# xavi-pinsach/kzg-grandsums-study

Hardware: AMD Instinct MI355X
Metric: grand-sum proofs/sec + MSM G1-adds/sec at n=2^20, 1/2/4/8 MI355X (higher is better)
Workload: dtype u32 limbs (BN254 Fr/Fq Montgomery: 8 x 32-bit; MSM buckets 9 x 29-bit), int VALU; 1 GPU; grandsum prover, n=2^20, k=1, no selectors, inputs resident in HBM; nbits=20, npols=1, selectors=False, parallelism=replicas x1, inflight_per_gpu=4, srs_power=20, srs_points_resident=2097151

## Files before the change

include/kgs.h:

```cpp
#ifndef KGS_H
#define KGS_H
#include <stddef.h>
#include <stdint.h>

#ifdef __cplusplus
extern "C" {
#endif

#define KGS_OK 0
#define KGS_E_ARG (-1)
#define KGS_E_HIP (-2)
#define KGS_E_NOT_WELL_CALC (-3)
#define KGS_E_NOT_DIVISIBLE (-4)
#define KGS_E_DOES_NOT_DIVIDE (-5)
#define KGS_E_IO (-6)
#define KGS_E_SRS (-7)
#define KGS_E_COMM (-8)
#define KGS_E_RANGE (-9)
#define KGS_E_NOT_IN_TABLE (-10)

#define KGS_GRANDSUM 0
#define KGS_GRANDPRODUCT 1
#define KGS_LOOKUP 2

// ... 3 lines not shown
const char* kgs_version(void);

int kgs_device_count(int* count);
int kgs_ctx_create(int device, kgs_ctx_t** out);
void kgs_ctx_destroy(kgs_ctx_t* ctx);

typedef int (*kgs_allgather_fn)(void* user, const uint8_t* send, uint8_t* recv, uint64_t bytes);
int kgs_ctx_set_shard(kgs_ctx_t* ctx, int rank, int world, kgs_allgather_fn fn, void* user);
int kgs_shard_range(uint64_t n, int rank, int world, uint64_t* lo, uint64_t* hi);
int kgs_msm_combine(const uint8_t* T_all, int nparts, int c, uint8_t out_lem[64]);

typedef struct kgs_group kgs_group_t;
int kgs_group_create_local(int world, kgs_group_t** out);
int kgs_group_create_host(int world, kgs_allgather_fn fn, void* user, kgs_group_t** out);
typedef int (*kgs_alltoall_fn)(void* user, const uint8_t* send, uint8_t* recv, uint64_t chunk);
int kgs_group_create_host_a2a(int world, kgs_allgather_fn fn, kgs_alltoall_fn a2a, void* user, kgs_group_t** out);
int kgs_group_rccl_unique_id(uint8_t id[128]);
int kgs_group_create_rccl(int rank, int world, const uint8_t id[128], int device, kgs_group_t** out);
void kgs_group_destroy(kgs_group_t* g);
int kgs_group_world(kgs_group_t* g, int* world);
int kgs_ctx_set_group(kgs_ctx_t* ctx, kgs_group_t* g, int rank);
int kgs_last_exchange(kgs_ctx_t* ctx, double* out, int max);

int kgs_ctx_set_msm_lanes(kgs_ctx_t* ctx, int lanes);

int kgs_ctx_set_reference_quirks(kgs_ctx_t* ctx, int on);

int kgs_srs_load_ptau(kgs_ctx_t* ctx, const char* path, int nbits_max);
int kgs_srs_load_ptau_slice(kgs_ctx_t* ctx, const char* path, int nbits_max, int rank, int world);
int kgs_srs_slice_info(kgs_ctx_t* ctx, int* rank, int* world, uint64_t* table_bytes);
int kgs_ptau_power(const char* path, int* power);
int kgs_srs_load_points(kgs_ctx_t* ctx, const uint8_t* g1_lem, uint64_t npts, int power, int nbits_max);
int kgs_srs_info(kgs_ctx_t* ctx, int* power, uint64_t* npts, int* window_c);
int kgs_ptau_read_tau_g2(const char* path, uint8_t out128[128]);

int kgs_ptau_write_synthetic(kgs_ctx_t* ctx, const char* path, int power, const uint8_t tau_std[32]);

int kgs_prove(kgs_ctx_t* ctx, int kind, int nbits, int npols, const uint8_t* const* evals_f,
              const uint8_t* const* evals_t, const uint8_t* sel_f, const uint8_t* sel_t, uint8_t* const* mont_f,
              uint8_t* const* mont_t, uint8_t* commitments_out, uint8_t* evaluations_out);
int kgs_host_register(void* ptr, uint64_t bytes);
int kgs_host_unregister(void* ptr);
int kgs_ctx_idle(kgs_ctx_t* ctx);
int kgs_prove_device(kgs_ctx_t* ctx, int kind, int nbits, int npols, const void* const* d_evals_f,
                     const void* const* d_evals_t, const void* d_sel_f, const void* d_sel_t, uint8_t* commitments_out,
                     uint8_t* evaluations_out);
int kgs_proof_shape(int kind, int npols, int selected, int* n_commitments, int* n_evaluations);

int kgs_verify(int kind, int nbits, int npols, int selected, const uint8_t* commitments, const uint8_t* evaluations,
               const uint8_t tau_g2[128]);
int kgs_verify_ptau(int kind, const char* ptau_path, int nbits, int npols, int selected, const uint8_t* commitments,
                    const uint8_t* evaluations);
int kgs_pairing_eq(int npairs, const uint8_t* g1_lem, const uint8_t* g2_lem);

typedef struct {
  int kind, nbits, npols, selected;
  const uint8_t* commitments;
  const uint8_t* evaluations;
} kgs_proof_ref_t;
typedef struct {
  uint8_t* weights_out;
  uint8_t* folded_out;
  uint32_t pairing_checks;
  uint32_t terms;
  int on_gpu;
  double fold_ms, pairing_ms;
// ... 85 lines not shown
```

kzg-grandsums-study_amd/csrc/field29.hpp:

```cpp
#pragma once
#include "field.hpp"

#ifndef KGS_M32_ROWS
#define KGS_M32_ROWS 8
#endif
#ifndef KGS_M32_ROWS_MUL2
#define KGS_M32_ROWS_MUL2 8
#endif
static_assert(KGS_M32_ROWS <= 8 && KGS_M32_ROWS_MUL2 <= 8, "column bounds of fq29::reduce_row32");

namespace kgs {
namespace f29 {

constexpr uint32_t MASK = 0x1fffffffu;
constexpr uint32_t INV = 0x04866389u;
constexpr uint32_t INV32 = 0x24866389u;
struct L9 {
  uint32_t v[9];
};
constexpr L9 Q = {{0x187cfd47u, 0x010460b6u, 0x1c72a34fu, 0x02d522d0u, 0x1585d978u, 0x02db40c0u, 0x00a6e141u,
                   0x0e5c2634u, 0x0030644eu}};
constexpr L9 ONE = {{0x157ccc21u, 0x141c2758u, 0x185230d3u, 0x014c0419u, 0x0aa36fb9u, 0x1d4240ceu, 0x11d54c07u,
                     0x052ac7a8u, 0x000dc836u}};
constexpr L9 C256 = {{0x058f0d9du, 0x1aea1c6eu, 0x11c2cf74u, 0x11d651ebu, 0x1462c0a7u, 0x11b7bc3cu, 0x1cbd99bau,
// ... 185 lines not shown
      const int64_t s = (int64_t)(Kc.v[j] - b.l[j]) + (int64_t)x.t[j] + c;
      r.l[j] = j < 8 ? ((uint32_t)s & f29::MASK) : (uint32_t)s;
      c = s >> 29;
    }
    return r;
  }

  __device__ __forceinline__ static fq29 mul(const fq29& a, const fq29& b) { return carry(mul_cols(a, b)); }
  __device__ __forceinline__ static fq29 sqr(const fq29& a) { return carry(sqr_cols(a)); }
  __device__ __forceinline__ static fq29 mul2(const fq29& a, const fq29& b, const fq29& c2, const fq29& d2) {
    return carry(mul2_cols(a, b, c2, d2));
  }

  __device__ __forceinline__ bool maybe_zero8() const {
    return ((l[0] * (0u - f29::INV)) & f29::MASK) < 8u;
  }
  __device__ __forceinline__ fq to_fq() const {
    fq29 m = mul(*this, from(f29::C256));
    fq r;
    m.pack(r.v);
    return fq::reduce_once(r);
  }
  __device__ __forceinline__ static fq29 from_fq(const fq& a) { return mul(unpack(a.v), from(f29::C266)); }
};

constexpr int RAW29_WORDS = 40;

struct g1_acc29 {
  fq29 X, Y, ZZ, ZZZ;
  bool inf;

  __device__ __forceinline__ void set_inf() { inf = true; }

  __device__ __forceinline__ void add_aff(const uint32_t* xw, const uint32_t* yw, bool negy) {
    uint32_t z = 0;
#pragma unroll
    for (int i = 0; i < 8; i++) z |= xw[i] | yw[i];
    if (z == 0) return;
    const fq29 x2 = fq29::unpack(xw), y2 = fq29::unpack(yw);
    if (inf) {
      X = x2;
      const fq29 yn = fq29::neg<2, 1>(y2).norm();
#pragma unroll
      for (int j = 0; j < 9; j++) Y.l[j] = negy ? yn.l[j] : y2.l[j];
      ZZ = fq29::from(f29::ONE);
      ZZZ = ZZ;
      inf = false;
      return;
    }
    const fq29 P = fq29::carry_sub<30, 1>(fq29::mul_cols(x2, ZZ), X);
    const fq29 S2 = fq29::mul(y2, ZZZ);
    fq29 R = fq29::neg<32, 2>(Y);
#pragma unroll
    for (int j = 0; j < 9; j++) R.l[j] = negy ? R.l[j] - S2.l[j] : R.l[j] + S2.l[j];
    R = R.norm();
    const fq29 PP = fq29::sqr(P);
    if (PP.maybe_zero8()) {
      if (P.to_fq().is_zero()) {
        if (R.to_fq().is_zero()) {
          g1_aff a;
          a.x = x2.to_fq();
          a.y = y2.to_fq();
          if (negy) a.y = a.y.neg();
          const g1_xyzz d = g1_xyzz::dbl_aff(a);
          X = fq29::from_fq(d.X);
          Y = fq29::from_fq(d.Y);
          ZZ = fq29::from_fq(d.ZZ);
          ZZZ = fq29::from_fq(d.ZZZ);
        } else {
          inf = true;
        }
// ... 100 lines not shown
```

kzg-grandsums-study_amd/csrc/kernels.hpp:

```cpp
#pragma once

#ifndef KGS_NO_PRIO_AUX
#define KGS_AUX_PRIO() __builtin_amdgcn_s_setprio(3)
#else
#define KGS_AUX_PRIO() ((void)0)
#endif

#include <hip/hip_runtime.h>
#include <stdint.h>
#include "field.hpp"

namespace kgs {

constexpr int LC_MAX = 32;
constexpr int LC_W29 = 10;
struct LinComb {
  int nterms;
  const uint32_t* src[LC_MAX];
  uint64_t len[LC_MAX];
  uint32_t coef[LC_MAX][8];
  uint32_t coef29[LC_MAX][LC_W29];
  uint32_t c0[8];
};

constexpr int EB_MAX = 32;
struct EvalBatch {
  int npolys;
  const uint32_t* src[EB_MAX];
  uint64_t len[EB_MAX];
};

struct MsmTables {
  uint32_t* table = nullptr;
  uint64_t npts = 0;
  int c = 0, W = 0;
};

constexpr int MSM_SL_G_MAX = 128;
constexpr int MSM_NH_MAX = 2048;
inline int msm_lob(int c) {
  int lob = c - 1 < 7 ? c - 1 : 7;
  if (c - 9 > lob) lob = c - 9 > 8 ? 8 : c - 9;
  return lob;
}
inline int msm_nh(int c) { return (1 << (c - 1)) >> msm_lob(c); }
struct MsmWork {
  int32_t* digit = nullptr;
  uint8_t* lo = nullptr;
  uint32_t* blockhist = nullptr;
  uint32_t *counts = nullptr, *offsets = nullptr, *cursor = nullptr, *sorted = nullptr;
  uint32_t* part = nullptr;
  uint32_t* segowner = nullptr;
  uint32_t* locnt = nullptr;
  uint32_t* chunklist = nullptr;
  uint32_t* chunkcnt = nullptr;
  uint32_t* raw29 = nullptr;
};

bool ntt_set_coresident(bool on);
constexpr int TW29_WORDS = 10;
void ntt_register_tw29(const uint32_t* base, uint64_t count, const uint32_t* twin);
void ntt_unregister_tw29(const uint32_t* base);
void launch_tw29(hipStream_t st, uint32_t* out, const uint32_t* in, uint64_t count);
void ntt_dif(hipStream_t st, uint32_t* out, const uint32_t* in, uint64_t in_len, int logm, const uint32_t* pre,
             const uint32_t* tw, int logM);
void ntt_dit(hipStream_t st, uint32_t* out, const uint32_t* in, int in_bitrev, int logm, const uint32_t* tw, int logM,
             const uint32_t* post, const uint32_t* post_s);
void launch_powers(hipStream_t st, uint32_t* out, uint64_t count, const uint32_t* w_dev, const uint32_t* scale_dev);
// ... 40 lines not shown
                           uint64_t N, uint64_t rot);
void launch_ref_divzh(hipStream_t st, uint32_t* c, uint64_t n, uint32_t ext, uint32_t* flag);

void launch_gather_e(hipStream_t st, uint32_t* out, const uint32_t* in, uint64_t N, int W, int r, bool to_mont);
void launch_dfwd_pack(hipStream_t st, uint32_t* send, const uint32_t* Z, int logMl, int W, int r, const uint32_t* tw,
                      int logN);
void launch_dfwd_wdft(hipStream_t st, uint32_t* out, const uint32_t* recv, int logMl, int W, const uint32_t* tw, int logN);
void launch_dinv_wdft_pack(hipStream_t st, uint32_t* send, const uint32_t* loc, int logMl, int W, int r,
                           const uint32_t* tw_inv, int logN);
void launch_unpack_c2b(hipStream_t st, uint32_t* out, const uint32_t* recv, uint64_t Lb, int W);
void launch_pack_b2c(hipStream_t st, uint32_t* send, const uint32_t* blk, uint64_t Lb, int W);
void launch_scan_fix(hipStream_t st, bool prod, uint32_t* out, const uint32_t* off, uint64_t n);
void launch_e_heads(hipStream_t st, uint32_t* heads, const uint32_t* S, uint64_t Ml, int W, int rot);
void launch_quotient_e(hipStream_t st, bool prod, bool sel, uint32_t* q, const uint32_t* S, const uint32_t* F,
                       const uint32_t* T, const uint32_t* SF, const uint32_t* ST, const uint32_t* nxm1,
                       const uint32_t* scalars, const uint32_t* halo, uint64_t Ml, int W, int r, int rot);
void launch_nxm1_e(hipStream_t st, uint32_t* out, const uint32_t* tw, int lcs, const uint32_t* gp, const uint32_t* np,
                   int W, int r);
void launch_div_fix(hipStream_t st, uint32_t* q, const uint32_t* pz, const uint32_t* c, uint64_t Lb);

struct LookupCols {
  int k;
  const uint32_t* col[EB_MAX];
};
void launch_lookup_multiplicities(hipStream_t st, uint32_t* out, uint32_t* table, uint64_t capacity, uint32_t* count,
                                  uint32_t* flags, const LookupCols& F, const LookupCols& T, const uint32_t* sel_f,
                                  uint64_t n);

void launch_g1_fold(hipStream_t st, uint32_t* out_aff, const uint32_t* points, const uint32_t* scalars,
                    const uint32_t* seg_off, uint64_t nterms, uint64_t nseg, uint32_t* term_xyzz, uint32_t* seg_xyzz,
                    uint32_t* scratch);

void msm_build_table(hipStream_t st, uint32_t* table, uint64_t npts, int c, int W, uint32_t* tmp_xyzz,
                     uint32_t* scratch);
void msm_run(hipStream_t st, const MsmTables& tb, MsmWork& w, const uint32_t* scalars, uint64_t N, uint32_t* T_out,
             hipEvent_t* ev = nullptr, uint64_t pbase = 0, uint64_t pstride = 1, bool exclusive_acc = false);
constexpr int MSM_POINTS_C_MIN = 7, MSM_POINTS_C_MAX = 16;
struct MsmPointsSizes {
  uint64_t digit, sorted, lo, blockhist, counts, offsets, cursor, segowner, locnt, chunklist, raw29, part, T;
};
MsmPointsSizes msm_points_sizes(uint64_t N, int c);
void msm_points_row29(hipStream_t st, uint32_t* row, uint64_t N);
void msm_points_run(hipStream_t st, MsmWork& w, const uint32_t* row29, const uint32_t* scalars_std, uint64_t N, int c,
                    uint32_t* T_out);
void launch_fixed_base(hipStream_t st, uint32_t* out_xyzz, const uint32_t* sc, uint64_t count, const uint32_t* tbl);
void launch_batch_affine(hipStream_t st, uint32_t* out_aff, const uint32_t* in_xyzz, uint32_t* scratch, uint64_t npts);

}
```

kzg-grandsums-study_amd/csrc/msm.hip:

```cpp
#include "kernels.hpp"
#include "field29.hpp"

namespace kgs {

static inline unsigned nb(uint64_t work, unsigned bs = 256) { return (unsigned)((work + bs - 1) / bs); }
constexpr int NH_MAX = MSM_NH_MAX;

__global__ void __launch_bounds__(256) k_tab_dbl(uint32_t* __restrict__ tmp, const uint32_t* __restrict__ prev,
                                                 uint64_t npts, int c) {
  KGS_AUX_PRIO();
  const uint64_t i = (uint64_t)blockIdx.x * blockDim.x + threadIdx.x;
  if (i >= npts) return;
  g1_aff a = g1_aff::load(prev + 16 * i);
  g1_xyzz r = g1_xyzz::from_aff(a);
  for (int k = 0; k < c; k++) r = r.dbl();
  r.store(tmp + 32 * i);
}

template <int CH>
__global__ void __launch_bounds__(256) k_batch_affine(uint32_t* __restrict__ out, const uint32_t* __restrict__ in,
                                                      uint32_t* __restrict__ scratch, uint64_t npts) {
  KGS_AUX_PRIO();
  const uint64_t t = (uint64_t)blockIdx.x * blockDim.x + threadIdx.x;
  const uint64_t start = t * CH;
// ... 3 lines not shown
  for (uint64_t i = start; i < end; i++) {
    acc.store(scratch + 8 * i);
    fq zz = fq::load(in + 32 * i + 16), zzz = fq::load(in + 32 * i + 24);
    if (!zz.is_zero()) acc = acc * (zz * zzz);
  }
  fq inv = acc.inverse();
  for (uint64_t i = end; i-- > start;) {
    fq zz = fq::load(in + 32 * i + 16), zzz = fq::load(in + 32 * i + 24);
    if (zz.is_zero()) {
      fq::zero().store(out + 16 * i);
      fq::zero().store(out + 16 * i + 8);
      continue;
    }
    fq pre = fq::load(scratch + 8 * i);
    fq zinv = inv * pre;
    inv = inv * (zz * zzz);
    fq x = fq::load(in + 32 * i) * (zinv * zzz);
    fq y = fq::load(in + 32 * i + 8) * (zinv * zz);
    x.store(out + 16 * i);
    y.store(out + 16 * i + 8);
  }
}

__global__ void __launch_bounds__(256) k_tab_to29(uint32_t* __restrict__ table, uint64_t nelem) {
  KGS_AUX_PRIO();
  const uint64_t i = (uint64_t)blockIdx.x * blockDim.x + threadIdx.x;
  if (i >= nelem) return;
  fq c;
#pragma unroll
  for (int k = 0; k < 8; k++) c.v[k] = f29::C261W[k];
  (fq::load(table + 8 * i) * c).store(table + 8 * i);
}

void msm_build_table(hipStream_t st, uint32_t* table, uint64_t npts, int c, int W, uint32_t* tmp_xyzz,
                     uint32_t* scratch) {
  for (int j = 1; j < W; j++) {
    const uint32_t* prev = table + (uint64_t)(j - 1) * npts * 16;
    uint32_t* cur = table + (uint64_t)j * npts * 16;
    hipLaunchKernelGGL(k_tab_dbl, dim3(nb(npts)), dim3(256), 0, st, tmp_xyzz, prev, npts, c);
    hipLaunchKernelGGL(k_batch_affine<32>, dim3(nb((npts + 31) / 32)), dim3(256), 0, st, cur, tmp_xyzz,
                       scratch, npts);
  }
  hipLaunchKernelGGL(k_tab_to29, dim3(nb(2 * (uint64_t)W * npts)), dim3(256), 0, st, table, 2 * (uint64_t)W * npts);
}

template <int C, bool STD = false, bool RED = false>
__device__ __forceinline__ void scalar_digits(int32_t (&d)[(255 + C - 1) / C], const uint32_t* sc, uint64_t i,
                                              uint32_t* std_out = nullptr) {
  constexpr int W = (255 + C - 1) / C;
  fr s = STD ? fr::load(sc + 8 * i) : fr::load(sc + 8 * i).from_mont();
  if (RED) {
#pragma unroll
    for (int k = 0; k < 5; k++) s = fr::reduce_once(s);
  }
  if (std_out) s.store(std_out + 8 * i);
  constexpr int32_t half = 1 << (C - 1);
  constexpr uint32_t mask = (1u << C) - 1;
  uint32_t carry = 0;
#pragma unroll
  for (int j = 0; j < W; j++) {
    const int bit = j * C;
    const int limb = bit >> 5, off = bit & 31;
    uint64_t w = limb < 8 ? s.v[limb] : 0;
    if (limb + 1 < 8) w |= (uint64_t)s.v[limb + 1] << 32;
    int32_t v = (int32_t)((w >> off) & mask) + (int32_t)carry;
    carry = v > half ? 1u : 0u;
    d[j] = carry ? v - (1 << C) : v;
  }
}

__device__ __forceinline__ uint32_t wave_excl_scan256(const uint32_t* a, uint32_t* out, int n) {
  const int lane = threadIdx.x & 63;
  uint32_t x[4], local = 0;
#pragma unroll
  for (int k = 0; k < 4; k++) {
    const int idx = lane * 4 + k;
    x[k] = idx < n ? a[idx] : 0;
    local += x[k];
  }
  uint32_t incl = local;
#pragma unroll
  for (int off = 1; off < 64; off <<= 1) {
    const uint32_t y = __shfl_up(incl, off);
// ... 30 lines not shown
    const uint32_t v = a[i];
    out[i] = run;
    run += v;
  }
  __syncthreads();
  return total;
}

__device__ __forceinline__ uint32_t part_of(uint32_t key, int lob) { return (key - 1) >> lob; }

template <int C, bool VAR>
__device__ __forceinline__ uint32_t sort_key(int j, uint32_t m) {
  return VAR ? (uint32_t)j * (1u << (C - 1)) + m : m;
}

#ifndef KGS_SORT_SPT
#define KGS_SORT_SPT 2
#endif
constexpr int SORT_SPT = KGS_SORT_SPT;

template <int C, bool VAR = false>
__global__ void __launch_bounds__(256) k_sort_hist(uint32_t* __restrict__ bh, const uint32_t* __restrict__ sc,
                                                   uint64_t N, int lob, int NH, uint32_t nblk,
                                                   uint32_t* __restrict__ std_out) {
  KGS_AUX_PRIO();
  constexpr int W = (255 + C - 1) / C;
  __shared__ uint32_t h[NH_MAX];
  for (int t = threadIdx.x; t < NH; t += 256) h[t] = 0;
  __syncthreads();
  for (int q = 0; q < SORT_SPT; q++) {
    const uint64_t i = ((uint64_t)blockIdx.x * SORT_SPT + q) * 256 + threadIdx.x;
    if (i < N) {
      int32_t d[W];
      if (VAR) scalar_digits<C, true, true>(d, sc, i, std_out);
      else scalar_digits<C>(d, sc, i, std_out);
#pragma unroll
      for (int j = 0; j < W; j++) {
        if (d[j]) atomicAdd(&h[part_of(sort_key<C, VAR>(j, (uint32_t)(d[j] < 0 ? -d[j] : d[j])), lob)], 1u);
      }
    }
  }
  __syncthreads();
  for (int t = threadIdx.x; t < NH; t += 256) bh[(uint64_t)t * nblk + blockIdx.x] = h[t];
}

__global__ void __launch_bounds__(256) k_sort_scan_blocks(uint32_t* __restrict__ bh, uint32_t* __restrict__ ptot,
                                                          uint32_t nblk) {
  KGS_AUX_PRIO();
  __shared__ uint32_t part[256];
  uint32_t* row = bh + (uint64_t)blockIdx.x * nblk;
  const uint32_t per = (nblk + 255) / 256;
  const uint32_t lo = threadIdx.x * per, hi = lo + per < nblk ? lo + per : nblk;
  uint32_t s = 0;
  for (uint32_t b = lo; b < hi; b++) s += row[b];
  part[threadIdx.x] = s;
  __syncthreads();
  for (int off = 1; off < 256; off <<= 1) {
    uint32_t v = threadIdx.x >= off ? part[threadIdx.x - off] : 0;
    __syncthreads();
    part[threadIdx.x] += v;
    __syncthreads();
  }
  uint32_t run = threadIdx.x ? part[threadIdx.x - 1] : 0;
  for (uint32_t b = lo; b < hi; b++) {
    uint32_t v = row[b];
    row[b] = run;
    run += v;
  }
// ... 25 lines not shown

template <int C, bool VAR = false>
__global__ void __launch_bounds__(256) k_sort_part(uint32_t* __restrict__ tval, uint8_t* __restrict__ tlo,
                                                   const uint32_t* __restrict__ bh, const uint32_t* __restrict__ ptot,
                                                   const uint32_t* __restrict__ hi_off, const uint32_t* __restrict__ sc,
                                                   uint64_t N, uint64_t Nsrs, uint64_t pbase, uint64_t pstride, int lob,
                                                   int NH, uint32_t nblk) {
  KGS_AUX_PRIO();
  constexpr int W = (255 + C - 1) / C;
  extern __shared__ uint32_t smem[];
  constexpr int NS = 256 * SORT_SPT * W;
  uint32_t* sval = smem;
  uint32_t* base = smem + NS;
  uint32_t* loff = base + NH;
  uint32_t* cur = loff + NH;
  uint16_t* spart = (uint16_t*)(cur + NH);
  uint8_t* slo = (uint8_t*)(spart + NS);
  __shared__ uint32_t tmp[256];
  const uint32_t blk = blockIdx.x, tid = threadIdx.x;
  for (int t = tid; t < NH; t += 256) {
    const uint32_t mine = bh[(uint64_t)t * nblk + blk];
    const uint32_t nxt = blk + 1 < nblk ? bh[(uint64_t)t * nblk + blk + 1] : ptot[t];
    base[t] = hi_off[t] + mine;
    cur[t] = nxt - mine;
  }
  __syncthreads();
  const uint32_t tot = block_excl_scan<256>(cur, loff, NH, tmp);
  for (int t = tid; t < NH; t += 256) cur[t] = loff[t];
  __syncthreads();
  for (int q = 0; q < SORT_SPT; q++) {
    const uint64_t i = ((uint64_t)blk * SORT_SPT + q) * 256 + tid;
    if (i < N) {
      int32_t d[W];
      scalar_digits<C, true>(d, sc, i);
      const uint32_t pidx = (uint32_t)pbase + (uint32_t)pstride * (uint32_t)i;
#pragma unroll
      for (int j = 0; j < W; j++) {
        if (!d[j]) continue;
        const uint32_t k = sort_key<C, VAR>(j, (uint32_t)(d[j] < 0 ? -d[j] : d[j]));
        const uint32_t p = part_of(k, lob);
        const uint32_t pos = atomicAdd(&cur[p], 1u);
        sval[pos] = (VAR ? (uint32_t)i : (uint32_t)j * (uint32_t)Nsrs + pidx) | (d[j] < 0 ? 0x80000000u : 0u);
        spart[pos] = (uint16_t)p;
        slo[pos] = (uint8_t)((k - 1) - (p << lob));
      }
    }
  }
  __syncthreads();
  for (uint32_t e = tid; e < tot; e += 256) {
    const uint32_t p = spart[e];
    const uint32_t g = base[p] + (e - loff[p]);
    tval[g] = sval[e];
    tlo[g] = slo[e];
  }
}

#ifndef KGS_SL_THREADS
#define KGS_SL_THREADS 1024
#endif
#ifndef KGS_SL_CHUNK
#define KGS_SL_CHUNK 16384
#endif
#ifndef KGS_SL_G
#define KGS_SL_G 64
#endif
constexpr int SL_THREADS = KGS_SL_THREADS;
constexpr int SL_TILE = KGS_SL_CHUNK;
// ... 226 lines not shown
    o[1] = rt0;
    o[2] = rt1;
    o[3] = (unsigned long long)__smid() | ((unsigned long long)blockIdx.x << 32);
  }
#endif
}

constexpr uint32_t CB_T = 16;
constexpr int CB_LEVELS = 3;

__device__ __forceinline__ void combine_enqueue(uint32_t* list, uint32_t* cnt, uint64_t s, uint64_t o0, uint64_t o1,
                                                uint32_t L, uint64_t stride) {
  if (s * L <= o0) return;
  const uint64_t s_lo = o0 / L + 1, s_hi = (o1 + L - 1) / L;
  if (s_hi - s_lo <= CB_T) return;
  if ((s - s_lo) % (stride * CB_T) != 0 || s + stride >= s_hi) return;
  list[atomicAdd(cnt, 1u)] = (uint32_t)s;
}

__device__ __forceinline__ uint32_t* run_rec(uint32_t* raw, uint64_t i) { return raw + RAW29_WORDS * i; }
__device__ __forceinline__ const uint32_t* run_rec(const uint32_t* raw, uint64_t i) { return raw + RAW29_WORDS * i; }

#ifndef KGS_ACC_WAVES
#define KGS_ACC_WAVES 2
#endif
#ifndef KGS_DIAG_GATHER_MASK
#define KGS_DIAG_GATHER_MASK 0x7fffffffu
#endif
#ifdef KGS_DIAG_CLOCK
constexpr int KGS_CLK_BLOCKS = 8192;
__device__ unsigned long long g_kgs_clk[4 * KGS_CLK_BLOCKS];
__device__ unsigned int g_kgs_clk_cu[KGS_CLK_BLOCKS];
#endif
template <int VW>
__global__ void __launch_bounds__(256, VW) k_accumulate(uint32_t* __restrict__ segowner,
                                                    uint32_t* __restrict__ chunklist, uint32_t* __restrict__ chunkcnt,
                                                    const uint32_t* __restrict__ sorted,
                                                    const uint32_t* __restrict__ offsets, uint32_t nbins,
                                                    const uint32_t* __restrict__ table, uint32_t L,
                                                    uint32_t* __restrict__ raw, uint32_t prio_m1, uint32_t prio_m2) {
  if (VW == 2) asm volatile("; reserve v175 (176 VGPRs: two waves per SIMD)" ::: "v175");
  const uint64_t s = (uint64_t)blockIdx.x * blockDim.x + threadIdx.x;
  const uint64_t E = offsets[nbins];
  const uint64_t start = s * L;
  if (start >= E) return;
#ifdef KGS_DIAG_CLOCK
  unsigned long long clk0 = 0, rt0 = 0;
  if (threadIdx.x == 0) {
    clk0 = __builtin_amdgcn_s_memtime();
    rt0 = __builtin_amdgcn_s_memrealtime();
  }
#endif
  const uint64_t end = start + L < E ? start + L : E;
  uint32_t lo = 0, hi = nbins;
  while (hi - lo > 1) {
    uint32_t mid = (lo + hi) >> 1;
    if (offsets[mid] <= start) lo = mid; else hi = mid;
  }
  uint32_t b = lo;
  const uint32_t o0 = offsets[b], o1 = offsets[b + 1];
  segowner[s] = b;
  combine_enqueue(chunklist, chunkcnt, s, o0, o1, L, 1);
  g1_acc29 acc;
  acc.set_inf();
  const uint32_t end32 = (uint32_t)end, last = end32 - 1;
  uint32_t rec = (uint32_t)start == o0 ? b : nbins + (uint32_t)s;
  uint32_t bend32 = o1, bnext = offsets[b + 2 <= nbins ? b + 2 : nbins];
  uint32_t v = sorted[start];
  uint32_t vn = sorted[start + 1 <= last ? start + 1 : last];
  const uint4* pt = reinterpret_cast<const uint4*>(table + 16 * (uint64_t)(v & KGS_DIAG_GATHER_MASK));
  uint4 a0 = pt[0], a1 = pt[1], a2 = pt[2], a3 = pt[3];
  uint32_t it = 0;
  if (prio_m1) __builtin_amdgcn_s_setprio(2);
  for (uint32_t e = (uint32_t)start; e <= last; e++, it++) {
    if (it == prio_m1) __builtin_amdgcn_s_setprio(1);
    if (it == prio_m2) __builtin_amdgcn_s_setprio(0);
    const uint4* pn = reinterpret_cast<const uint4*>(table + 16 * (uint64_t)(vn & KGS_DIAG_GATHER_MASK));
    const uint4 n0 = pn[0], n1 = pn[1], n2 = pn[2], n3 = pn[3];
    const uint32_t vnn = sorted[e + 2 <= last ? e + 2 : last];
    if (e >= bend32) {
      acc.store_raw(run_rec(raw, rec));
      b++;
      bend32 = bnext;
      while (e >= bend32) {
        b++;
        bend32 = offsets[b + 1];
      }
      rec = b;
      acc.set_inf();
    }
    bnext = offsets[b + 2 <= nbins ? b + 2 : nbins];
    const uint32_t xw[8] = {a0.x, a0.y, a0.z, a0.w, a1.x, a1.y, a1.z, a1.w};
    const uint32_t yw[8] = {a2.x, a2.y, a2.z, a2.w, a3.x, a3.y, a3.z, a3.w};
    acc.add_aff(xw, yw, (v & 0x80000000u) != 0);
    a0 = n0; a1 = n1; a2 = n2; a3 = n3;
    v = vn;
    vn = vnn;
  }
  acc.store_raw(run_rec(raw, rec));
#ifdef KGS_DIAG_CLOCK
  if (threadIdx.x == 0 && blockIdx.x < KGS_CLK_BLOCKS) {
    const unsigned long long clk1 = __builtin_amdgcn_s_memtime(), rt1 = __builtin_amdgcn_s_memrealtime();
    unsigned long long* o = g_kgs_clk + 4 * blockIdx.x;
    o[0] = clk0;
    o[1] = clk1;
    o[2] = rt0;
    o[3] = rt1;
    unsigned int xcc;
    asm volatile("s_getreg_b32 %0, hwreg(HW_REG_XCC_ID)" : "=s"(xcc));
    g_kgs_clk_cu[blockIdx.x] = ((xcc & 15u) << 16) | (unsigned int)__smid();
  }
#endif
}

#ifdef KGS_DIAG_CLOCK
extern "C" int kgs_diag_lorec(unsigned long long* out, unsigned int cap, unsigned int* n, int reset) {
  if (hipDeviceSynchronize() != hipSuccess) return 1;
  unsigned int cnt = 0;
  if (hipMemcpyFromSymbol(&cnt, HIP_SYMBOL(g_kgs_lorec_n), sizeof(cnt)) != hipSuccess) return 1;
  const unsigned int have = cnt < KGS_LOREC_CAP ? cnt : KGS_LOREC_CAP;
  const unsigned int m = have < cap ? have : cap;
  if (m && hipMemcpyFromSymbol(out, HIP_SYMBOL(g_kgs_lorec), 32ull * m) != hipSuccess) return 1;
  *n = m;
  if (reset) {
    const unsigned int z = 0;
    if (hipMemcpyToSymbol(HIP_SYMBOL(g_kgs_lorec_n), &z, sizeof(z)) != hipSuccess) return 1;
  }
// ... 139 lines not shown
    for (uint32_t t = j; t < n; t += RC_LANES) {
      const uint32_t b = row ? (line << l) | t : (t << l) | (line - (1u << h));
      if (b) v.add(g1_acc29::load_raw(run_rec(raw, b)));
    }
  }
#pragma unroll
  for (int m = RC_LANES / 2; m >= 1; m >>= 1) v.add(shfl_xor_acc(v, m));
  if (line < nlines && j == 0) v.store_raw(rc + (uint64_t)RAW29_WORDS * line);
}

__global__ void __launch_bounds__(128) k_bitsum_rc(uint32_t* __restrict__ T, const uint32_t* __restrict__ rc,
                                                   const uint32_t* __restrict__ raw, int c) {
  KGS_AUX_PRIO();
  __shared__ __attribute__((aligned(16))) uint32_t lds[64 * RAW29_WORDS];
  const int l = c / 2, h = c - 1 - l;
  const int k = blockIdx.x;
  const uint32_t t = threadIdx.x;
  g1_acc29 v;
  v.set_inf();
  if (k == c - 1) {
    if (t == 0) v = g1_acc29::load_raw(run_rec(raw, 1u << (c - 1)));
  } else {
    const int bits = k < l ? l : h, j = k < l ? k : k - l;
    const uint32_t base = k < l ? 1u << h : 0u;
    for (uint32_t e = t; e < (1u << (bits - 1)); e += 128) {
      const uint32_t idx = ((e >> j) << (j + 1)) | (1u << j) | (e & ((1u << j) - 1));
      v.add(g1_acc29::load_raw(rc + (uint64_t)RAW29_WORDS * (base + idx)));
    }
  }
  v = block_tree_sum(v, lds);
  if (t == 0) v.to_xyzz().store(T + 32 * (uint64_t)k);
}

static void msm_buckets(hipStream_t st, MsmWork& w, const uint32_t* table, uint64_t E, int NH, int lob, uint32_t B,
                        bool exclusive_acc, hipEvent_t* ev) {
  uint32_t* hi_off = w.cursor;
  uint32_t* cpre = w.cursor + NH_MAX + 8;
  uint32_t* bpart = w.cursor + 2 * (NH_MAX + 8);
  const uint64_t chunk_bound = std::min<uint64_t>((uint64_t)NH * SL_G, NH + E / SL_CHUNK);
  hipLaunchKernelGGL(k_lo_count, dim3((unsigned)chunk_bound), dim3(LC_THREADS), 0, st, w.locnt, w.lo, hi_off, cpre,
                     bpart, NH, lob);
  hipLaunchKernelGGL(k_lo_scatter, dim3((unsigned)chunk_bound), dim3(SL_THREADS), 0, st, w.sorted, w.offsets, w.locnt,
                     (const uint32_t*)w.digit, w.lo, hi_off, cpre, bpart, NH, lob);
  if (ev) hipEventRecord(ev[1], st);
  static const int cus = [] {
    int dev = 0, n = 0;
    if (hipGetDevice(&dev) != hipSuccess || hipDeviceGetAttribute(&n, hipDeviceAttributeMultiprocessorCount, dev) != hipSuccess || n <= 0) n = 256;
    return n;
  }();
  const uint64_t resident = (uint64_t)cus * KGS_ACC_WAVES * 256;
  uint64_t L = (E + resident - 1) / resident;
  if (L < 4) L = 4;
  if ((E + L - 1) / L > (1ull << 18)) L = (E + (1ull << 18) - 1) >> 18;
  const uint64_t nseg = (E + L - 1) / L;
  uint32_t* cnt = w.chunkcnt;
  const uint64_t lcap = nseg / CB_T + B + 16;
  hipMemsetAsync(cnt, 0, 4 * CB_LEVELS, st);
  static const int acc_prio = [] {
    const char* e = getenv("KGS_ACC_PRIO");
    return e ? atoi(e) : 1;
  }();
#ifdef KGS_NO_PRIO_AUX
  const bool prio = false;
  (void)acc_prio;
#else
  const bool prio = acc_prio >= 2 || (acc_prio == 1 && exclusive_acc);
#endif
  const uint32_t pm1 = prio ? (uint32_t)(3 * L / 4) : 0u, pm2 = prio ? (uint32_t)(93 * L / 100) : 0u;
  if (exclusive_acc)
    hipLaunchKernelGGL(k_accumulate<2>, dim3(nb(nseg)), dim3(256), 0, st, w.segowner, w.chunklist, cnt, w.sorted,
                       w.offsets, B + 1, table, (uint32_t)L, w.raw29, pm1, pm2);
  else
    hipLaunchKernelGGL(k_accumulate<3>, dim3(nb(nseg)), dim3(256), 0, st, w.segowner, w.chunklist, cnt, w.sorted,
                       w.offsets, B + 1, table, (uint32_t)L, w.raw29, pm1, pm2);
  if (ev) hipEventRecord(ev[2], st);
  uint64_t stride = 1, cap = lcap;
  for (int j = 0; j < CB_LEVELS; j++, stride *= CB_T) {
    uint32_t* lin = w.chunklist + (uint64_t)j * lcap;
    uint32_t* lout = j + 1 < CB_LEVELS ? w.chunklist + (uint64_t)(j + 1) * lcap : nullptr;
    hipLaunchKernelGGL(k_combine_level, dim3(nb(cap)), dim3(256), 0, st, w.raw29, B + 1, w.segowner, w.offsets, lin,
                       cnt + j, lout, lout ? cnt + j + 1 : nullptr, (uint32_t)L, stride);
    cap = cap / CB_T + B + 16;
  }
  hipLaunchKernelGGL(k_combine, dim3(nb(COMBINE_LANES * (uint64_t)B)), dim3(256), 0, st, w.raw29, B + 1, w.offsets, B,
                     (uint32_t)L, stride);
}

void msm_run(hipStream_t st, const MsmTables& tb, MsmWork& w, const uint32_t* scalars, uint64_t N,
             uint32_t* T_out, hipEvent_t* ev, uint64_t pbase, uint64_t pstride, bool exclusive_acc) {
  if (ev) hipEventRecord(ev[0], st);
  const int c = tb.c, W = tb.W;
  const uint32_t B = 1u << (c - 1);
  const int lob = msm_lob(c);
  const int NH = (int)(B >> lob);
  const uint32_t nblk = (uint32_t)((N + 256 * SORT_SPT - 1) / (256 * SORT_SPT));
  uint32_t* ptot = w.counts;
  uint32_t* hi_off = w.cursor;
  uint32_t* cpre = w.cursor + NH_MAX + 8;
  uint32_t* bpart = w.cursor + 2 * (NH_MAX + 8);
  uint32_t* bh = w.blockhist;
  const size_t part_lds = (size_t)256 * SORT_SPT * W * 7 + (size_t)12 * NH;
  uint32_t* scal_std = w.sorted;
  switch (c) {
#define KGS_SORT_C(CC)                                                                                         \
  case CC:                                                                                                      \
    hipLaunchKernelGGL(k_sort_hist<CC>, dim3(nblk), dim3(256), 0, st, bh, scalars, N, lob, NH, nblk, scal_std); \
    hipLaunchKernelGGL(k_sort_scan_blocks, dim3(NH), dim3(256), 0, st, bh, ptot, nblk);                       \
    hipLaunchKernelGGL(k_sort_scan, dim3(1), dim3(256), 0, st, hi_off, ptot, NH, w.offsets, B, cpre, bpart); \
    hipLaunchKernelGGL(k_sort_part<CC>, dim3(nblk), dim3(256), part_lds, st, (uint32_t*)w.digit, w.lo, bh,   \
                       ptot, hi_off, scal_std, N, tb.npts, pbase, pstride, lob, NH, nblk);                    \
    break;
    KGS_SORT_C(7) KGS_SORT_C(8) KGS_SORT_C(9) KGS_SORT_C(10) KGS_SORT_C(11) KGS_SORT_C(12)
    KGS_SORT_C(13) KGS_SORT_C(14) KGS_SORT_C(15) KGS_SORT_C(16) KGS_SORT_C(17) KGS_SORT_C(18)
    KGS_SORT_C(19) KGS_SORT_C(20)
#undef KGS_SORT_C
    default:
      return;
  }
  msm_buckets(st, w, tb.table, N * (uint64_t)W, NH, lob, B, exclusive_acc, ev);
  if (ev) hipEventRecord(ev[3], st);
  const uint32_t nlines = (1u << (c - 1 - c / 2)) + (1u << (c / 2));
#ifndef KGS_ROWCOL16
#define KGS_ROWCOL16 1
#endif
  if (exclusive_acc || !KGS_ROWCOL16)
    hipLaunchKernelGGL(k_rowcol, dim3(nlines), dim3(256), 0, st, w.part, w.raw29, c);
  else
    hipLaunchKernelGGL(k_rowcol16, dim3((nlines * RC_LANES + 255) / 256), dim3(256), 0, st, w.part, w.raw29, c);
  hipLaunchKernelGGL(k_bitsum_rc, dim3(c), dim3(128), 0, st, T_out, w.part, w.raw29, c);
  if (ev) hipEventRecord(ev[4], st);
}

__global__ void __launch_bounds__(256) k_rowcol_win(uint32_t* __restrict__ rc, const uint32_t* __restrict__ raw, int c) {
  KGS_AUX_PRIO();
  __shared__ __attribute__((aligned(16))) uint32_t lds[128 * RAW29_WORDS];
  const int l = c / 2, h = c - 1 - l;
  const uint32_t r = blockIdx.x, t = threadIdx.x, win = blockIdx.y;
  const uint32_t nlines = (1u << h) + (1u << l);
  raw += (uint64_t)RAW29_WORDS * win * (1u << (c - 1));
  const bool row = r < (1u << h);
  g1_acc29 v;
  v.set_inf();
  const uint32_t n = row ? 1u << l : 1u << h;
  for (uint32_t e = t; e < n; e += 256) {
    const uint32_t b = row ? (r << l) | e : (e << l) | (r - (1u << h));
    if (b) v.add(g1_acc29::load_raw(run_rec(raw, b)));
  }
  v = block_tree_sum(v, lds);
  if (t == 0) v.store_raw(rc + (uint64_t)RAW29_WORDS * (win * nlines + r));
}

__global__ void __launch_bounds__(256) k_rowcol16_win(uint32_t* __restrict__ rc, const uint32_t* __restrict__ raw,
// ... 79 lines not shown
  if (N) hipLaunchKernelGGL(k_tab_to29, dim3(nb(2 * N)), dim3(256), 0, st, row, 2 * N);
}

void msm_points_run(hipStream_t st, MsmWork& w, const uint32_t* row29, const uint32_t* scalars_std, uint64_t N, int c,
                    uint32_t* T_out) {
  const int W = (255 + c - 1) / c;
  const uint32_t B = (uint32_t)W << (c - 1);
  const int cs = points_c_sort(c);
  const int lob = msm_lob(cs), NH = msm_nh(cs);
  const uint32_t nblk = (uint32_t)((N + 256 * SORT_SPT - 1) / (256 * SORT_SPT));
  uint32_t* ptot = w.counts;
  uint32_t* hi_off = w.cursor;
  uint32_t* cpre = w.cursor + NH_MAX + 8;
  uint32_t* bpart = w.cursor + 2 * (NH_MAX + 8);
  uint32_t* bh = w.blockhist;
  const size_t part_lds = (size_t)256 * SORT_SPT * W * 7 + (size_t)12 * NH;
  uint32_t* scal_std = w.sorted;
  switch (c) {
#define KGS_SORT_C(CC)                                                                                               \
  case CC:                                                                                                            \
    hipLaunchKernelGGL((k_sort_hist<CC, true>), dim3(nblk), dim3(256), 0, st, bh, scalars_std, N, lob, NH, nblk,      \
                       scal_std);                                                                                     \
    hipLaunchKernelGGL(k_sort_scan_blocks, dim3(NH), dim3(256), 0, st, bh, ptot, nblk);                               \
    hipLaunchKernelGGL(k_sort_scan, dim3(1), dim3(256), 0, st, hi_off, ptot, NH, w.offsets, B, cpre, bpart);          \
    hipLaunchKernelGGL((k_sort_part<CC, true>), dim3(nblk), dim3(256), part_lds, st, (uint32_t*)w.digit, w.lo, bh,    \
                       ptot, hi_off, scal_std, N, (uint64_t)0, (uint64_t)0, (uint64_t)0, lob, NH, nblk);              \
    break;
    KGS_SORT_C(7) KGS_SORT_C(8) KGS_SORT_C(9) KGS_SORT_C(10) KGS_SORT_C(11) KGS_SORT_C(12)
    KGS_SORT_C(13) KGS_SORT_C(14) KGS_SORT_C(15) KGS_SORT_C(16)
#undef KGS_SORT_C
    default:
      return;
  }
  msm_buckets(st, w, row29, N * (uint64_t)W, NH, lob, B, false, nullptr);
  const uint32_t nlines = (1u << (c - 1 - c / 2)) + (1u << (c / 2));
  if (!KGS_ROWCOL16)
    hipLaunchKernelGGL(k_rowcol_win, dim3(nlines, W), dim3(256), 0, st, w.part, w.raw29, c);
  else
    hipLaunchKernelGGL(k_rowcol16_win, dim3((nlines * RC_LANES + 255) / 256, W), dim3(256), 0, st, w.part, w.raw29, c);
  hipLaunchKernelGGL(k_bitsum_rc_win, dim3(c, W), dim3(128), 0, st, T_out, w.part, w.raw29, c);
}

__global__ void __launch_bounds__(256) k_fixed_base(uint32_t* __restrict__ out_xyzz, const uint32_t* __restrict__ sc,
                                                    uint64_t count, const uint32_t* __restrict__ tbl) {
  KGS_AUX_PRIO();
  const uint64_t i = (uint64_t)blockIdx.x * blockDim.x + threadIdx.x;
  if (i >= count) return;
  fr s = fr::load(sc + 8 * i).from_mont();
  g1_xyzz acc = g1_xyzz::inf();
  for (int j = 0; j < 32; j++) {
    uint32_t d = (s.v[j >> 2] >> ((j & 3) * 8)) & 0xffu;
    if (d) acc.add_aff(g1_aff::load(tbl + 16 * ((uint64_t)j * 256 + d)));
  }
  acc.store(out_xyzz + 32 * i);
}

void launch_fixed_base(hipStream_t st, uint32_t* out_xyzz, const uint32_t* sc, uint64_t count, const uint32_t* tbl) {
  hipLaunchKernelGGL(k_fixed_base, dim3(nb(count)), dim3(256), 0, st, out_xyzz, sc, count, tbl);
}

void launch_batch_affine(hipStream_t st, uint32_t* out_aff, const uint32_t* in_xyzz, uint32_t* scratch, uint64_t npts) {
  hipLaunchKernelGGL(k_batch_affine<32>, dim3(nb((npts + 31) / 32)), dim3(256), 0, st, out_aff, in_xyzz, scratch, npts);
}

}
```

kzg-grandsums-study_amd/csrc/prover.cpp:

```cpp
#include <hip/hip_runtime.h>
#include <stdio.h>
#include <stdlib.h>
#include <string.h>
#include <chrono>
#include <algorithm>
#include <map>
#include <mutex>
#include <sys/stat.h>
#include <memory>
#include <stdexcept>
#include <string>
#include <functional>
#include <atomic>
#include <thread>
#include <immintrin.h>
#include <vector>

#include "../../include/kgs.h"
#include "host_field.hpp"
#include "host_pairing.hpp"
#include "kernels.hpp"
#include "host_error.hpp"
#ifndef KGS_NO_ROCTX
#include <rocprofiler-sdk-roctx/roctx.h>
// ... 196 lines not shown
  c.sync();
  c.use_srs(nullptr);
  c.work_npts = 0;
  std::shared_ptr<SrsTables> s;
  {
    std::lock_guard<std::mutex> lk(g_reg_mu);
    s = srs_lookup(c.device, file, nbits_max, srank, sworld);
  }
  if (!s) {
    int cc = choose_c(npts);
    int W = (255 + cc - 1) / cc;
    while ((uint64_t)W * npts > (1ull << 31) && cc < KGS_C_MAX) {
      cc++;
      W = (255 + cc - 1) / cc;
    }
    if ((uint64_t)W * npts > (1ull << 31)) throw KgsError(KGS_E_SRS, "SRS too large for the MSM entry index");
    auto t = std::make_shared<SrsTables>();
    t->device = c.device;
    t->file = file;
    t->power = power;
    t->nbits_max = nbits_max;
    t->slice_rank = srank;
    t->slice_world = sworld;
    t->tb.npts = npts;
    t->tb.c = cc;
    t->tb.W = W;
    HC(dev_malloc((void**)&t->tb.table, (size_t)W * npts * 64));
    HC(hipMemcpyAsync(t->tb.table, lem, npts * 64, hipMemcpyHostToDevice, c.st));
    struct Tmp {
      void* p = nullptr;
      ~Tmp() {
        if (p) hipFree(p);
      }
    } tmp, scr;
    HC(dev_malloc(&tmp.p, npts * 128));
    HC(dev_malloc(&scr.p, npts * 32));
    msm_build_table(c.st, t->tb.table, npts, cc, W, (uint32_t*)tmp.p, (uint32_t*)scr.p);
    check_launch();
    HC(hipStreamSynchronize(c.st));
    std::lock_guard<std::mutex> lk(g_reg_mu);
    if (auto other = srs_lookup(c.device, file, nbits_max, srank, sworld)) {
      s = other;
    } else {
      g_srs_reg.erase(std::remove_if(g_srs_reg.begin(), g_srs_reg.end(), [](auto& w) { return w.expired(); }),
                      g_srs_reg.end());
      if (!file.empty()) g_srs_reg.push_back(t);
      s = t;
    }
  }
  ensure_domain(c, s->nbits_max + 1);
  MsmTables keep = c.tb;
  c.tb = s->tb;
  try {
    ensure_msm_work(c);
  } catch (...) {
    c.tb = keep;
    c.use_srs(nullptr);
    throw;
  }
  c.sync();
  c.use_srs(s);
}


hipStream_t copy_stream() {
  static const bool low = [] {
    const char* e = getenv("KGS_COPY_STREAM_PRIO");
    return !(e && !strcmp(e, "normal"));
  }();
  hipStream_t s = nullptr;
  if (low) {
    int least = 0, greatest = 0;
// ... 494 lines not shown
}

extern "C" {

int kgs_srs_load_ptau(kgs_ctx_t* ctx, const char* path, int nbits_max) {
  API_BEGIN
  load_ptau_impl(ctx, path, nbits_max, 0, 1);
  API_END
}

int kgs_srs_load_ptau_slice(kgs_ctx_t* ctx, const char* path, int nbits_max, int rank, int world) {
  API_BEGIN
  load_ptau_impl(ctx, path, nbits_max, rank, world);
  API_END
}

int kgs_srs_slice_info(kgs_ctx_t* ctx, int* rank, int* world, uint64_t* table_bytes) {
  API_BEGIN
  if (!ctx) throw KgsError(KGS_E_ARG, "NULL ctx");
  CTX_LOCK(ctx);
  if (rank) *rank = ctx->srs_slice_rank;
  if (world) *world = ctx->srs_slice_world;
  if (table_bytes) *table_bytes = ctx->srs ? (uint64_t)ctx->tb.W * ctx->tb.npts * 64 : 0;
  API_END
}

int kgs_srs_info(kgs_ctx_t* ctx, int* power, uint64_t* npts, int* window_c) {
  API_BEGIN
  if (!ctx) throw KgsError(KGS_E_ARG, "NULL ctx");
  CTX_LOCK(ctx);
  if (power) *power = ctx->srs_power;
  if (npts) *npts = ctx->tb.npts;
  if (window_c) *window_c = ctx->tb.c;
  API_END
}

int kgs_ptau_write_synthetic(kgs_ctx_t* ctx, const char* path, int power, const uint8_t tau_std[32]) {
  API_BEGIN
  if (!path || !tau_std || power < 1 || power > 28) throw KgsError(KGS_E_ARG, "bad argument");
  uint64_t s[4];
  memcpy(s, tau_std, 32);
  Fr tau = Fr::from_std(s);
  const uint64_t n1 = (1ull << (power + 1)) - 1;
  std::vector<uint8_t> g1(n1 * 64);
  std::vector<uint8_t> tbl = g1_fixed_table();
  if (ctx) {
    CTX_LOCK(ctx);
    HC(hipSetDevice(ctx->device));
    ctx->reset_staging();
    uint32_t* d_tau = ctx->scal(&tau, 1);
    uint32_t* pw = ctx->buf("syn_pow", 32 * n1);
    uint32_t* xy = ctx->buf("syn_xyzz", 128 * n1);
    uint32_t* scr = ctx->buf("syn_scr", 32 * n1);
    uint32_t* aff = ctx->buf("syn_aff", 64 * n1);
    uint32_t* dtbl = ctx->buf("syn_tbl", tbl.size());
    HC(hipMemcpyAsync(dtbl, tbl.data(), tbl.size(), hipMemcpyHostToDevice, ctx->st));
    launch_powers(ctx->st, pw, n1, d_tau, nullptr);
    launch_fixed_base(ctx->st, xy, pw, n1, dtbl);
    launch_batch_affine(ctx->st, aff, xy, scr, n1);
    check_launch();
    HC(hipMemcpyAsync(g1.data(), aff, g1.size(), hipMemcpyDeviceToHost, ctx->st));
    ctx->reset_staging();
  } else {
    Fr t = Fr::one();
    for (uint64_t i = 0; i < n1; i++) {
      uint64_t e[4];
// ... 1090 lines not shown
```

Before: 95.60 proofs/s.

## Fold Montgomery factor into SRS table and skip zero-point checks in MSM

At SRS table build time, each base point is multiplied by the scalar R^-1 (Montgomery inverse) on device. This lets the MSM digit extraction use Montgomery-form scalars directly and drop the per-scalar from_mont conversion and the std-scalar scratch write in sort_hist/sort_part. The build also records whether any point is at infinity. When none is, the accumulate kernel is instantiated without the per-add zero check. The trade is a more expensive one-time table build and extra template instantiations.

```diff
diff --git a/include/kgs.h b/include/kgs.h
--- a/include/kgs.h
+++ b/include/kgs.h
@@ -59,6 +59,7 @@
 int kgs_ptau_power(const char* path, int* power);
 int kgs_srs_load_points(kgs_ctx_t* ctx, const uint8_t* g1_lem, uint64_t npts, int power, int nbits_max);
 int kgs_srs_info(kgs_ctx_t* ctx, int* power, uint64_t* npts, int* window_c);
+int kgs_srs_zero_points(kgs_ctx_t* ctx, int* zero_points);
 int kgs_ptau_read_tau_g2(const char* path, uint8_t out128[128]);
 
 int kgs_ptau_write_synthetic(kgs_ctx_t* ctx, const char* path, int power, const uint8_t tau_std[32]);
diff --git a/kzg-grandsums-study_amd/csrc/field29.hpp b/kzg-grandsums-study_amd/csrc/field29.hpp
--- a/kzg-grandsums-study_amd/csrc/field29.hpp
+++ b/kzg-grandsums-study_amd/csrc/field29.hpp
@@ -241,11 +241,14 @@
 
   __device__ __forceinline__ void set_inf() { inf = true; }
 
+  template <bool ZP = true>
   __device__ __forceinline__ void add_aff(const uint32_t* xw, const uint32_t* yw, bool negy) {
-    uint32_t z = 0;
-#pragma unroll
-    for (int i = 0; i < 8; i++) z |= xw[i] | yw[i];
-    if (z == 0) return;
+    if (ZP) {
+      uint32_t z = 0;
+#pragma unroll
+      for (int i = 0; i < 8; i++) z |= xw[i] | yw[i];
+      if (z == 0) return;
+    }
     const fq29 x2 = fq29::unpack(xw), y2 = fq29::unpack(yw);
     if (inf) {
       X = x2;
diff --git a/kzg-grandsums-study_amd/csrc/kernels.hpp b/kzg-grandsums-study_amd/csrc/kernels.hpp
--- a/kzg-grandsums-study_amd/csrc/kernels.hpp
+++ b/kzg-grandsums-study_amd/csrc/kernels.hpp
@@ -34,6 +34,7 @@
   uint32_t* table = nullptr;
   uint64_t npts = 0;
   int c = 0, W = 0;
+  bool zero_points = true;
 };
 
 constexpr int MSM_SL_G_MAX = 128;
@@ -140,7 +141,7 @@
                     uint32_t* scratch);
 
 void msm_build_table(hipStream_t st, uint32_t* table, uint64_t npts, int c, int W, uint32_t* tmp_xyzz,
-                     uint32_t* scratch);
+                     uint32_t* scratch, const uint32_t rho[8], uint32_t* zero_flag);
 void msm_run(hipStream_t st, const MsmTables& tb, MsmWork& w, const uint32_t* scalars, uint64_t N, uint32_t* T_out,
              hipEvent_t* ev = nullptr, uint64_t pbase = 0, uint64_t pstride = 1, bool exclusive_acc = false);
 constexpr int MSM_POINTS_C_MIN = 7, MSM_POINTS_C_MAX = 16;
diff --git a/kzg-grandsums-study_amd/csrc/msm.hip b/kzg-grandsums-study_amd/csrc/msm.hip
--- a/kzg-grandsums-study_amd/csrc/msm.hip
+++ b/kzg-grandsums-study_amd/csrc/msm.hip
@@ -59,8 +59,39 @@
   (fq::load(table + 8 * i) * c).store(table + 8 * i);
 }
 
+struct MsmScalar {
+  uint32_t w[8];
+};
+__global__ void __launch_bounds__(256) k_tab_scale(uint32_t* __restrict__ tmp, const uint32_t* __restrict__ row0,
+                                                   uint64_t npts, MsmScalar rho, int top,
+                                                   uint32_t* __restrict__ zero_flag) {
+  KGS_AUX_PRIO();
+  const uint64_t i = (uint64_t)blockIdx.x * blockDim.x + threadIdx.x;
+  if (i >= npts) return;
+  const g1_aff a = g1_aff::load(row0 + 16 * i);
+  if (a.is_inf()) *zero_flag = 1u;
+  g1_xyzz r = g1_xyzz::from_aff(a);
+  for (int k = top - 1; k >= 0; k--) {
+    r = r.dbl();
+    if ((rho.w[k >> 5] >> (k & 31)) & 1u) r.add_aff(a);
+  }
+  r.store(tmp + 32 * i);
+}
+
 void msm_build_table(hipStream_t st, uint32_t* table, uint64_t npts, int c, int W, uint32_t* tmp_xyzz,
-                     uint32_t* scratch) {
+                     uint32_t* scratch, const uint32_t rho[8], uint32_t* zero_flag) {
+  MsmScalar k;
+  int top = -1;
+  for (int b = 0; b < 8; b++) k.w[b] = rho[b];
+  for (int b = 0; b < 256; b++) {
+    if ((rho[b >> 5] >> (b & 31)) & 1u) top = b;
+  }
+  hipMemsetAsync(zero_flag, 0, 4, st);
+  if (top >= 0) {
+    hipLaunchKernelGGL(k_tab_scale, dim3(nb(npts)), dim3(256), 0, st, tmp_xyzz, table, npts, k, top, zero_flag);
+    hipLaunchKernelGGL(k_batch_affine<32>, dim3(nb((npts + 31) / 32)), dim3(256), 0, st, table, tmp_xyzz, scratch,
+                       npts);
+  }
   for (int j = 1; j < W; j++) {
     const uint32_t* prev = table + (uint64_t)(j - 1) * npts * 16;
     uint32_t* cur = table + (uint64_t)j * npts * 16;
@@ -71,11 +102,11 @@
   hipLaunchKernelGGL(k_tab_to29, dim3(nb(2 * (uint64_t)W * npts)), dim3(256), 0, st, table, 2 * (uint64_t)W * npts);
 }
 
-template <int C, bool STD = false, bool RED = false>
+template <int C, bool RED = false>
 __device__ __forceinline__ void scalar_digits(int32_t (&d)[(255 + C - 1) / C], const uint32_t* sc, uint64_t i,
                                               uint32_t* std_out = nullptr) {
   constexpr int W = (255 + C - 1) / C;
-  fr s = STD ? fr::load(sc + 8 * i) : fr::load(sc + 8 * i).from_mont();
+  fr s = fr::load(sc + 8 * i);
   if (RED) {
 #pragma unroll
     for (int k = 0; k < 5; k++) s = fr::reduce_once(s);
@@ -172,8 +203,8 @@
     const uint64_t i = ((uint64_t)blockIdx.x * SORT_SPT + q) * 256 + threadIdx.x;
     if (i < N) {
       int32_t d[W];
-      if (VAR) scalar_digits<C, true, true>(d, sc, i, std_out);
-      else scalar_digits<C>(d, sc, i, std_out);
+      if (VAR) scalar_digits<C, true>(d, sc, i, std_out);
+      else scalar_digits<C>(d, sc, i);
 #pragma unroll
       for (int j = 0; j < W; j++) {
         if (d[j]) atomicAdd(&h[part_of(sort_key<C, VAR>(j, (uint32_t)(d[j] < 0 ? -d[j] : d[j])), lob)], 1u);
@@ -265,7 +296,7 @@
     const uint64_t i = ((uint64_t)blk * SORT_SPT + q) * 256 + tid;
     if (i < N) {
       int32_t d[W];
-      scalar_digits<C, true>(d, sc, i);
+      scalar_digits<C>(d, sc, i);
       const uint32_t pidx = (uint32_t)pbase + (uint32_t)pstride * (uint32_t)i;
 #pragma unroll
       for (int j = 0; j < W; j++) {
@@ -558,7 +589,7 @@
 __device__ unsigned long long g_kgs_clk[4 * KGS_CLK_BLOCKS];
 __device__ unsigned int g_kgs_clk_cu[KGS_CLK_BLOCKS];
 #endif
-template <int VW>
+template <int VW, bool ZP>
 __global__ void __launch_bounds__(256, VW) k_accumulate(uint32_t* __restrict__ segowner,
                                                     uint32_t* __restrict__ chunklist, uint32_t* __restrict__ chunkcnt,
                                                     const uint32_t* __restrict__ sorted,
@@ -618,7 +649,7 @@
     bnext = offsets[b + 2 <= nbins ? b + 2 : nbins];
     const uint32_t xw[8] = {a0.x, a0.y, a0.z, a0.w, a1.x, a1.y, a1.z, a1.w};
     const uint32_t yw[8] = {a2.x, a2.y, a2.z, a2.w, a3.x, a3.y, a3.z, a3.w};
-    acc.add_aff(xw, yw, (v & 0x80000000u) != 0);
+    acc.add_aff<ZP>(xw, yw, (v & 0x80000000u) != 0);
     a0 = n0; a1 = n1; a2 = n2; a3 = n3;
     v = vn;
     vn = vnn;
@@ -824,8 +855,8 @@
   if (t == 0) v.to_xyzz().store(T + 32 * (uint64_t)k);
 }
 
-static void msm_buckets(hipStream_t st, MsmWork& w, const uint32_t* table, uint64_t E, int NH, int lob, uint32_t B,
-                        bool exclusive_acc, hipEvent_t* ev) {
+static void msm_buckets(hipStream_t st, MsmWork& w, const uint32_t* table, bool zero_points, uint64_t E, int NH,
+                        int lob, uint32_t B, bool exclusive_acc, hipEvent_t* ev) {
   uint32_t* hi_off = w.cursor;
   uint32_t* cpre = w.cursor + NH_MAX + 8;
   uint32_t* bpart = w.cursor + 2 * (NH_MAX + 8);
@@ -859,12 +890,17 @@
   const bool prio = acc_prio >= 2 || (acc_prio == 1 && exclusive_acc);
 #endif
   const uint32_t pm1 = prio ? (uint32_t)(3 * L / 4) : 0u, pm2 = prio ? (uint32_t)(93 * L / 100) : 0u;
-  if (exclusive_acc)
-    hipLaunchKernelGGL(k_accumulate<2>, dim3(nb(nseg)), dim3(256), 0, st, w.segowner, w.chunklist, cnt, w.sorted,
-                       w.offsets, B + 1, table, (uint32_t)L, w.raw29, pm1, pm2);
-  else
-    hipLaunchKernelGGL(k_accumulate<3>, dim3(nb(nseg)), dim3(256), 0, st, w.segowner, w.chunklist, cnt, w.sorted,
-                       w.offsets, B + 1, table, (uint32_t)L, w.raw29, pm1, pm2);
+#define KGS_ACC(VW, ZP)                                                                                        \
+  hipLaunchKernelGGL((k_accumulate<VW, ZP>), dim3(nb(nseg)), dim3(256), 0, st, w.segowner, w.chunklist, cnt,   \
+                     w.sorted, w.offsets, B + 1, table, (uint32_t)L, w.raw29, pm1, pm2)
+  if (exclusive_acc) {
+    if (zero_points) KGS_ACC(2, true);
+    else KGS_ACC(2, false);
+  } else {
+    if (zero_points) KGS_ACC(3, true);
+    else KGS_ACC(3, false);
+  }
+#undef KGS_ACC
   if (ev) hipEventRecord(ev[2], st);
   uint64_t stride = 1, cap = lcap;
   for (int j = 0; j < CB_LEVELS; j++, stride *= CB_T) {
@@ -892,15 +928,15 @@
   uint32_t* bpart = w.cursor + 2 * (NH_MAX + 8);
   uint32_t* bh = w.blockhist;
   const size_t part_lds = (size_t)256 * SORT_SPT * W * 7 + (size_t)12 * NH;
-  uint32_t* scal_std = w.sorted;
   switch (c) {
 #define KGS_SORT_C(CC)                                                                                         \
   case CC:                                                                                                      \
-    hipLaunchKernelGGL(k_sort_hist<CC>, dim3(nblk), dim3(256), 0, st, bh, scalars, N, lob, NH, nblk, scal_std); \
+    hipLaunchKernelGGL(k_sort_hist<CC>, dim3(nblk), dim3(256), 0, st, bh, scalars, N, lob, NH, nblk,          \
+                       (uint32_t*)nullptr);                                                                     \
     hipLaunchKernelGGL(k_sort_scan_blocks, dim3(NH), dim3(256), 0, st, bh, ptot, nblk);                       \
     hipLaunchKernelGGL(k_sort_scan, dim3(1), dim3(256), 0, st, hi_off, ptot, NH, w.offsets, B, cpre, bpart); \
     hipLaunchKernelGGL(k_sort_part<CC>, dim3(nblk), dim3(256), part_lds, st, (uint32_t*)w.digit, w.lo, bh,   \
-                       ptot, hi_off, scal_std, N, tb.npts, pbase, pstride, lob, NH, nblk);                    \
+                       ptot, hi_off, scalars, N, tb.npts, pbase, pstride, lob, NH, nblk);                     \
     break;
     KGS_SORT_C(7) KGS_SORT_C(8) KGS_SORT_C(9) KGS_SORT_C(10) KGS_SORT_C(11) KGS_SORT_C(12)
     KGS_SORT_C(13) KGS_SORT_C(14) KGS_SORT_C(15) KGS_SORT_C(16) KGS_SORT_C(17) KGS_SORT_C(18)
@@ -909,7 +945,7 @@
     default:
       return;
   }
-  msm_buckets(st, w, tb.table, N * (uint64_t)W, NH, lob, B, exclusive_acc, ev);
+  msm_buckets(st, w, tb.table, tb.zero_points, N * (uint64_t)W, NH, lob, B, exclusive_acc, ev);
   if (ev) hipEventRecord(ev[3], st);
   const uint32_t nlines = (1u << (c - 1 - c / 2)) + (1u << (c / 2));
 #ifndef KGS_ROWCOL16
@@ -1055,7 +1091,7 @@
     default:
       return;
   }
-  msm_buckets(st, w, row29, N * (uint64_t)W, NH, lob, B, false, nullptr);
+  msm_buckets(st, w, row29, true, N * (uint64_t)W, NH, lob, B, false, nullptr);
   const uint32_t nlines = (1u << (c - 1 - c / 2)) + (1u << (c / 2));
   if (!KGS_ROWCOL16)
     hipLaunchKernelGGL(k_rowcol_win, dim3(nlines, W), dim3(256), 0, st, w.part, w.raw29, c);
diff --git a/kzg-grandsums-study_amd/csrc/prover.cpp b/kzg-grandsums-study_amd/csrc/prover.cpp
--- a/kzg-grandsums-study_amd/csrc/prover.cpp
+++ b/kzg-grandsums-study_amd/csrc/prover.cpp
@@ -252,12 +252,22 @@
       ~Tmp() {
         if (p) hipFree(p);
       }
-    } tmp, scr;
+    } tmp, scr, zflag;
     HC(dev_malloc(&tmp.p, npts * 128));
     HC(dev_malloc(&scr.p, npts * 32));
-    msm_build_table(c.st, t->tb.table, npts, cc, W, (uint32_t*)tmp.p, (uint32_t*)scr.p);
+    HC(dev_malloc(&zflag.p, 16));
+    host::Fr rinv = host::Fr::zero();
+    rinv.v[0] = 1;
+    uint64_t rho64[4];
+    rinv.to_std(rho64);
+    uint32_t rho[8];
+    memcpy(rho, rho64, 32);
+    msm_build_table(c.st, t->tb.table, npts, cc, W, (uint32_t*)tmp.p, (uint32_t*)scr.p, rho, (uint32_t*)zflag.p);
     check_launch();
+    uint32_t zero_points = 1;
+    HC(hipMemcpyAsync(&zero_points, zflag.p, 4, hipMemcpyDeviceToHost, c.st));
     HC(hipStreamSynchronize(c.st));
+    t->tb.zero_points = zero_points != 0;
     std::lock_guard<std::mutex> lk(g_reg_mu);
     if (auto other = srs_lookup(c.device, file, nbits_max, srank, sworld)) {
       s = other;
@@ -818,6 +828,14 @@
   if (power) *power = ctx->srs_power;
   if (npts) *npts = ctx->tb.npts;
   if (window_c) *window_c = ctx->tb.c;
+  API_END
+}
+
+int kgs_srs_zero_points(kgs_ctx_t* ctx, int* zero_points) {
+  API_BEGIN
+  if (!ctx || !zero_points) throw KgsError(KGS_E_ARG, "NULL argument");
+  CTX_LOCK(ctx);
+  *zero_points = ctx->srs ? (ctx->tb.zero_points ? 1 : 0) : -1;
   API_END
 }
 
diff --git a/profiles/valu_by_kernel.py b/profiles/valu_by_kernel.py
--- /dev/null
+++ b/profiles/valu_by_kernel.py
@@ -0,0 +1,42 @@
+#!/usr/bin/env python3
+import collections
+import csv
+import sys
+
+COUNTER = "SQ_INSTS_VALU"
+
+
+def totals(path, proofs):
+    tot, n = collections.Counter(), collections.Counter()
+    for r in csv.DictReader(open(path)):
+        if r["Counter_Name"] != COUNTER:
+            continue
+        name = r["Kernel_Name"].split("(")[0].replace("kgs::", "").replace("void ", "")
+        tot[name] += float(r["Counter_Value"]) / proofs / 1e6
+        n[name] += 1
+    return tot, n
+
+
+def main():
+    proofs = float(sys.argv[1])
+    a, na = totals(sys.argv[2], proofs)
+    b, nb = totals(sys.argv[3], proofs) if len(sys.argv) > 3 else (None, None)
+    base = lambda k: k.split("<")[0]
+    if b is None:
+        for k, v in sorted(a.items(), key=lambda kv: -kv[1]):
+            print(f"{v:12.3f} M  x{na[k] / proofs:7.1f}  {k}")
+        print(f"{sum(a.values()):12.3f} M  total")
+        return
+    ga, gb = collections.Counter(), collections.Counter()
+    for k, v in a.items():
+        ga[base(k)] += v
+    for k, v in b.items():
+        gb[base(k)] += v
+    print(f"{'before M':>12s} {'after M':>12s} {'delta M':>10s}  kernel")
+    for k in sorted(set(ga) | set(gb), key=lambda k: -max(ga[k], gb[k])):
+        print(f"{ga[k]:12.3f} {gb[k]:12.3f} {gb[k] - ga[k]:10.3f}  {k}")
+    print(f"{sum(ga.values()):12.3f} {sum(gb.values()):12.3f} {sum(gb.values()) - sum(ga.values()):10.3f}  total")
+
+
+if __name__ == "__main__":
+    main()
```

After: 96.68 proofs/s, median of 6. +1.1%, better.
